# yakvrz/minesweeper-ppo

Hardware: NVIDIA B200
Metric: env_steps_per_s (higher is better)
Workload: dtype u32

## Files before the change

minesweeper_ppo_b200/csrc/msw_env.cu:

```cuda
#include "../../include/msw_b200.h"
#include "msw_common.cuh"
#include "msw_error.h"

#include <cuda_runtime.h>
#include <stdint.h>
#include <stdlib.h>
#include <string.h>


namespace msw {

void expand_obs_host(int H, int W, const uint32_t *mines, const uint32_t *revealed, const int32_t *meta, long long n,
                     float *obs, uint8_t *mask, uint64_t *shadow, int shadow_valid, int threads);

struct EnvParams {
    int H, W, HW, wpb;
    int mine_count, safe;
    float r_step, r_loss, r_win;
    uint32_t k0, k1;
    uint32_t thresh16;
    long long env_id_base;
    long long n;
    uint32_t *mines, *revealed, *flags;
    int4 *meta;
    const int32_t *a32;
    const long long *a64;
    const uint32_t *inj_bits;
    const uint8_t *inj_sel;
    float *reward;
    uint8_t *done;
    int8_t *outcome;
    int32_t *new_reveals, *step, *rcount;
    float *obs;
    uint8_t *mask;
    float *labels;
    uint8_t *valid;
    int rand_mode;
    uint32_t rk0, rk1, rand_step;
    int32_t *a_out;
    int vec_mode;
    long long seg_wa, seg_na, seg_wb, seg_nb;
    uint32_t g_valid[32], g_notcol0[32], g_notlast[32];
};

enum { MODE_STEP = 0, MODE_RESET = 1, MODE_ENCODE = 2 };

template <int CW, int CHW>
__device__ __noinline__ uint32_t sample_mines(const EnvParams &p, long long env_id, uint32_t episode,
                                              uint32_t startmask, int lane, const Geo &g)
{
    const int W = CW ? CW : p.W;
    const int HW = CHW ? CHW : p.HW;
    const int wpb = (HW + 31) >> 5;
    const int M = p.mine_count;
    uint32_t forb = startmask;
    if (p.safe) forb |= dilate8<CW>(startmask, lane, W, g);
    int allowed = HW - warp_popc_sum(forb);
    if (allowed < M) {
        forb = startmask;
        allowed = HW - 1;
    }
    const bool comp = 2 * M > allowed;
    const int K = comp ? allowed - M : M;
    const uint32_t thresh = CHW ? (65536u % (uint32_t)(CHW ? CHW : 1)) : p.thresh16;
    const uint32_t id_lo = (uint32_t)(unsigned long long)env_id;
    const uint32_t id_hi = (uint32_t)((unsigned long long)env_id >> 32);
    const uint32_t lt_mask = (1u << lane) - 1u;

    uint32_t chosen = 0;
    int cnt = 0;
    for (uint32_t batch = 0; cnt < K; ++batch) {
        uint32_t w[4];
        philox4x32_10(p.k0, p.k1, id_lo, id_hi, episode, batch * 32u + (uint32_t)lane, w);
#pragma unroll
        for (int r = 0; r < 8; ++r) {
            if (cnt >= K) break;
            const uint32_t x = (w[r >> 1] >> (16 * (r & 1))) & 0xFFFFu;
            const uint32_t m = x * (uint32_t)HW;
            const uint32_t d = m >> 16;
            const int owner = (int)(d >> 5);
            const uint32_t bit = 1u << (d & 31u);
            const uint32_t occ = __shfl_sync(FULL, forb | chosen, owner);
            const bool cand = ((m & 0xFFFFu) >= thresh) && !(occ & bit);
            const uint32_t same = __match_any_sync(FULL, cand ? d : (0x10000u + (uint32_t)lane));
            const bool novel = cand && ((same & lt_mask) == 0u);
            const uint32_t B = __ballot_sync(FULL, novel);
            const int need = K - cnt;
            const bool keep = novel && (__popc(B & lt_mask) < need);
            const int got = __popc(B);
            cnt += got < need ? got : need;
            for (int wd = 0; wd < wpb; ++wd) {
                const uint32_t nb = __reduce_or_sync(FULL, (keep && owner == wd) ? bit : 0u);
                if (lane == wd) chosen |= nb;
            }
        }
    }
    return comp ? (g.valid & ~forb & ~chosen) : chosen;
}

template <int CW, int CHW>
__device__ __forceinline__ void encode_board(const EnvParams &p, long long b, int lane, uint32_t R,
                                             uint32_t M, uint32_t F, int first, const Planes &pl,
                                             const Geo &g, const float4 *__restrict__ lut)
{
    const int HW = CHW ? CHW : p.HW;
    if (p.vec_mode == 1) {
        const int quads = HW >> 2;
        float4 *obs_b = p.obs ? reinterpret_cast<float4 *>(p.obs + b * (long long)(MSW_OBS_CHANNELS * HW)) : nullptr;
        uint32_t *mask_b = p.mask ? reinterpret_cast<uint32_t *>(p.mask + b * (long long)HW) : nullptr;
        float4 *lab_b = p.labels ? reinterpret_cast<float4 *>(p.labels + b * (long long)HW) : nullptr;
        uint32_t *val_b = p.valid ? reinterpret_cast<uint32_t *>(p.valid + b * (long long)HW) : nullptr;
        const uint32_t gate = first ? 15u : 0u;
#pragma unroll 2
        for (int q0 = 0; q0 < quads; q0 += 32) {
            const int q = q0 + lane;
            const bool act = q < quads;
            const int src = (act ? q : 0) >> 3;
            const int sh = (q & 7) << 2;
            const uint32_t r4 = (__shfl_sync(FULL, R, src) >> sh) & 15u;
            const uint32_t a0 = __shfl_sync(FULL, pl.c0, src) >> sh;
            const uint32_t a1 = __shfl_sync(FULL, pl.c1, src) >> sh;
            const uint32_t a2 = __shfl_sync(FULL, pl.c2, src) >> sh;
            const uint32_t a3 = __shfl_sync(FULL, pl.c3, src) >> sh;
            uint32_t l4 = 0, f4 = 0;
            if (lab_b) l4 = (__shfl_sync(FULL, M, src) >> sh) & gate;
            if (val_b && p.flags) f4 = (__shfl_sync(FULL, F, src) >> sh) & 15u;
            if (!act) continue;
            const uint32_t n4 = r4 ^ 15u;
            if (obs_b) {
                const uint32_t g4 = r4 & gate;
                float4 *o = obs_b + q;
                __stcs(o, lut[r4]);
#pragma unroll
                for (int k = 0; k < 9; ++k) {
                    const uint32_t lo = g4 & ((k & 1) ? a0 : ~a0) & ((k & 2) ? a1 : ~a1);
                    const uint32_t m = lo & ((k & 4) ? a2 : ~a2) & ((k & 8) ? a3 : ~a3);
                    __stcs(o + (1 + k) * quads, lut[m]);
                }
            }
            if (mask_b) __stcs(mask_b + q, nib_to_b4(n4));
            if (lab_b) __stcs(lab_b + q, lut[l4]);
            if (val_b) __stcs(val_b + q, nib_to_b4(n4 & ~f4 & gate));
        }
    } else {
        const uint32_t Lm = first ? M : 0u;
        const uint32_t Vm = first ? (~R & ~F & g.valid) : 0u;
        const int wpb = (HW + 31) >> 5;
        float *obs_b = p.obs ? p.obs + b * (long long)(MSW_OBS_CHANNELS * HW) : nullptr;
        uint8_t *mask_b = p.mask ? p.mask + b * (long long)HW : nullptr;
        float *lab_b = p.labels ? p.labels + b * (long long)HW : nullptr;
        uint8_t *val_b = p.valid ? p.valid + b * (long long)HW : nullptr;
        for (int it = 0; it < wpb; ++it) {
            const int cell = it * 32 + lane;
            const uint32_t r = (__shfl_sync(FULL, R, it) >> lane) & 1u;
            const uint32_t cnt = ((__shfl_sync(FULL, pl.c0, it) >> lane) & 1u) |
                                 (((__shfl_sync(FULL, pl.c1, it) >> lane) & 1u) << 1) |
                                 (((__shfl_sync(FULL, pl.c2, it) >> lane) & 1u) << 2) |
// ... 490 lines not shown
    g.notcol0 = p.g_notcol0[lane];
    g.notlast = p.g_notlast[lane];
    for (long long b = (long long)blockIdx.x * warps_per_block + (threadIdx.x >> 5); b < p.n; b += total_warps) {
        uint32_t M = 0, R = 0, F = 0;
        if (lane < wpb) {
            M = p.mines[b * wpb + lane];
            R = p.revealed[b * wpb + lane];
            if (p.flags) F = p.flags[b * wpb + lane];
        }
        const Planes pl = count_planes<0>(M, lane, p.W, g);
        for (int it = 0; it < wpb; ++it) {
            const int cell = it * 32 + lane;
            const uint32_t m = (__shfl_sync(FULL, M, it) >> lane) & 1u;
            const uint32_t r = (__shfl_sync(FULL, R, it) >> lane) & 1u;
            const uint32_t f = (__shfl_sync(FULL, F, it) >> lane) & 1u;
            const uint32_t cnt = ((__shfl_sync(FULL, pl.c0, it) >> lane) & 1u) |
                                 (((__shfl_sync(FULL, pl.c1, it) >> lane) & 1u) << 1) |
                                 (((__shfl_sync(FULL, pl.c2, it) >> lane) & 1u) << 2) |
                                 (((__shfl_sync(FULL, pl.c3, it) >> lane) & 1u) << 3);
            if (cell >= HW) continue;
            const long long o = b * (long long)HW + cell;
            if (q.o_mine) q.o_mine[o] = (uint8_t)m;
            if (q.o_rev) q.o_rev[o] = (uint8_t)r;
            if (q.o_flags) q.o_flags[o] = (uint8_t)f;
            if (q.o_counts) q.o_counts[o] = (uint8_t)cnt;
        }
    }
}

struct ActParams {
    const uint32_t *revealed;
    int HW, wpb;
    long long n, env_id_base;
    uint32_t k0, k1, step_index;
    int valid_only;
    int32_t *a32;
    long long *a64;
};

__global__ void __launch_bounds__(256) random_actions_kernel(const ActParams p)
{
    const long long b = (long long)blockIdx.x * blockDim.x + threadIdx.x;
    if (b >= p.n) return;
    const unsigned long long id = (unsigned long long)(p.env_id_base + b);
    uint32_t w[4];
    philox4x32_10(p.k0, p.k1 ^ 0x41435431u, (uint32_t)id, (uint32_t)(id >> 32), p.step_index, 0x5eedac71u, w);
    int action = 0;
    if (!p.valid_only) {
        action = (int)bounded(w, (uint32_t)p.HW);
    } else {
        const uint32_t *R = p.revealed + b * p.wpb;
        int cnt = 0;
        for (int i = 0; i < p.wpb; ++i) {
            uint32_t valid = (i == p.wpb - 1 && (p.HW & 31)) ? ((1u << (p.HW & 31)) - 1u) : 0xffffffffu;
            cnt += __popc(~R[i] & valid);
        }
        if (cnt > 0) {
            int k = (int)bounded(w, (uint32_t)cnt);
            for (int i = 0; i < p.wpb; ++i) {
                uint32_t valid = (i == p.wpb - 1 && (p.HW & 31)) ? ((1u << (p.HW & 31)) - 1u) : 0xffffffffu;
                const uint32_t free_cells = ~R[i] & valid;
                const int c = __popc(free_cells);
                if (k < c) {
                    action = i * 32 + (int)__fns(free_cells, 0, k + 1);
                    break;
                }
                k -= c;
            }
        }
    }
    if (p.a32) p.a32[b] = action;
    if (p.a64) p.a64[b] = action;
}

static int fill_geometry(EnvParams &p, const msw_env_desc *d, long long n)
{
    if (!d) return fail(MSW_ERR_NULL, "desc is NULL");
    if (d->H < 1 || d->W < 1 || d->W > 32 || (long long)d->H * d->W > MSW_MAX_CELLS)
        return fail(MSW_ERR_BAD_SHAPE, "board %dx%d unsupported (need 1<=W<=32, H*W<=%d)", d->H, d->W, MSW_MAX_CELLS);
    if (d->mine_count < 0 || d->mine_count > d->H * d->W - 1)
        return fail(MSW_ERR_BAD_SHAPE, "mine_count %d out of range for %dx%d", d->mine_count, d->H, d->W);
    if (n < 0) return fail(MSW_ERR_BAD_SHAPE, "n=%lld < 0", n);
    memset(&p, 0, sizeof(p));
    p.H = d->H; p.W = d->W; p.HW = d->H * d->W; p.wpb = (p.HW + 31) / 32;
    p.mine_count = d->mine_count; p.safe = d->safe_nbhd != 0;
    p.r_step = d->reward_step; p.r_loss = d->reward_loss; p.r_win = d->reward_win;
    p.k0 = (uint32_t)d->seed; p.k1 = (uint32_t)(d->seed >> 32);
    p.thresh16 = 65536u % (uint32_t)p.HW;
    p.env_id_base = d->env_id_base;
    p.n = n;
    for (int w = 0; w < 32; ++w) {
        uint32_t v = 0, a = 0, z = 0;
        for (int j = 0; j < 32; ++j) {
            const int cell = w * 32 + j;
            if (cell >= p.HW) break;
            const int col = cell % p.W;
            v |= 1u << j;
            if (col != 0) a |= 1u << j;
            if (col != p.W - 1) z |= 1u << j;
        }
        p.g_valid[w] = v; p.g_notcol0[w] = a; p.g_notlast[w] = z;
    }
    return MSW_OK;
}

static int fill_params(EnvParams &p, const msw_env_desc *d, const msw_state *st, long long n)
{
    if (!st) return fail(MSW_ERR_NULL, "state is NULL");
    if (!st->mines || !st->revealed || !st->meta) return fail(MSW_ERR_NULL, "state pointer is NULL");
    if (((uintptr_t)st->meta & 15u) != 0) return fail(MSW_ERR_ALIGN, "state.meta must be 16-byte aligned");
    const int rc = fill_geometry(p, d, n);
    if (rc) return rc;
    p.mines = st->mines; p.revealed = st->revealed; p.flags = st->flags;
    p.meta = reinterpret_cast<int4 *>(st->meta);
    return MSW_OK;
}

static int set_encode_out(EnvParams &p, const msw_encode_out *out, bool require)
{
    if (!out) return require ? fail(MSW_ERR_NULL, "encode outputs are NULL") : MSW_OK;
    p.obs = out->obs; p.mask = out->mask; p.labels = out->mine_labels; p.valid = out->mine_valid;
    const uintptr_t f = (uintptr_t)p.obs | (uintptr_t)p.labels, m = (uintptr_t)p.mask | (uintptr_t)p.valid;
    p.vec_mode = 0;
    if ((p.HW & 3) == 0) {
        if ((f & 15u) || (m & 3u))
            return fail(MSW_ERR_ALIGN, "obs/mine_labels must be 16-byte and mask/mine_valid 4-byte aligned");
        p.vec_mode = 1;
    }
    return MSW_OK;
}

struct LaunchShape { int block, bpw; };

static inline LaunchShape launch_shape_cfg()
{
#ifdef MSW_DEV_KNOBS
    static const LaunchShape c = [] {
        auto env_int = [](const char *name, int dflt) { const char *e = getenv(name); return e ? atoi(e) : dflt; };
        LaunchShape v;
        int blk = env_int("MSW_BLOCK", 32);
        if (blk < 32) blk = 32;
        if (blk > 256) blk = 256;
        v.block = blk & ~31;
        v.bpw = env_int("MSW_BPW", 3);
        if (v.bpw < 1) v.bpw = 1;
        return v;
    }();
    return c;
#else
    return LaunchShape{32, 3};
#endif
}

static inline int grid_for(EnvParams &q, int resident_warps_per_sm, int *block_out)
{
    const LaunchShape c = launch_shape_cfg();
    const int wpc = c.block / 32;
    *block_out = c.block;
    const long long n = q.n;
    long long taper_pct = 200;
#ifdef MSW_DEV_KNOBS
    if (const char *e = getenv("MSW_TAPER_PCT")) taper_pct = atoll(e);
#endif
    const long long S = (long long)sm_count() * resident_warps_per_sm;
    long long n2 = 0, n1 = 0;
    if (c.bpw >= 3 && n >= 8 * S && taper_pct > 0) {
        n1 = S / 3 * taper_pct / 100;
        n2 = 2 * n1;
    }
    q.seg_na = n - n2 - n1;
    q.seg_wa = (q.seg_na + c.bpw - 1) / c.bpw;
    q.seg_nb = q.seg_na + n2;
    q.seg_wb = (n2 + 1) / 2;
    const long long warps = q.seg_wa + q.seg_wb + n1;
    long long blocks = (warps + wpc - 1) / wpc;
    if (blocks < 1) blocks = 1;
    if (blocks > 0x7fffffffLL) blocks = 0x7fffffffLL;
    return (int)blocks;
}

template <int MODE, int CW, int CHW>
static void launch_shape(const EnvParams &p, int grid, int block, cudaStream_t s)
{
    if (MODE != MODE_STEP)
        env_kernel<MODE, CW, CHW, false, 4><<<grid, block, 0, s>>>(p);
    else
        env_kernel<MODE, CW, CHW, true, 3><<<grid, block, 0, s>>>(p);
}

template <int MODE>
static int launch_env(const EnvParams &p_in, cudaStream_t s)
{
    if (p_in.n == 0) return MSW_OK;
    EnvParams p = p_in;
    int block = 256;
    const int grid = grid_for(p, MODE == MODE_STEP ? 24 : 32, &block);
    if (p.W == 16 && p.HW == 256)
        launch_shape<MODE, 16, 256>(p, grid, block, s);
    else if (p.W == 30 && p.HW == 480)
        launch_shape<MODE, 30, 480>(p, grid, block, s);
    else if (p.W == 16 && p.HW == 480)
        launch_shape<MODE, 16, 480>(p, grid, block, s);
    else
        launch_shape<MODE, 0, 0>(p, grid, block, s);
    MSW_CUDA_TRY(cudaGetLastError());
    return MSW_OK;
}

}

using namespace msw;

extern "C" int msw_reset(const msw_env_desc *desc, const msw_state *st, int64_t n,
                         const msw_encode_out *out, void *stream)
{
    EnvParams p;
    int rc = fill_params(p, desc, st, n);
    if (rc) return rc;
    if ((rc = set_encode_out(p, out, false))) return rc;
    return launch_env<MODE_RESET>(p, (cudaStream_t)stream);
}

extern "C" int msw_encode(const msw_env_desc *desc, const msw_state *st, int64_t n,
                          const msw_encode_out *out, void *stream)
{
    EnvParams p;
    int rc = fill_params(p, desc, st, n);
    if (rc) return rc;
    if ((rc = set_encode_out(p, out, true))) return rc;
    return launch_env<MODE_ENCODE>(p, (cudaStream_t)stream);
}

static int fill_step(EnvParams &p, const msw_env_desc *desc, const msw_state *st, const msw_step_io *io, int64_t n)
{
    int rc = fill_params(p, desc, st, n);
    if (rc) return rc;
    if (!io) return fail(MSW_ERR_NULL, "io is NULL");
    if (io->rand_mode < 0 || io->rand_mode > 2) return fail(MSW_ERR_ARG, "rand_mode must be 0, 1 or 2");
    if (!io->rand_mode && (io->actions32 != nullptr) == (io->actions64 != nullptr))
        return fail(MSW_ERR_ARG, "exactly one of actions32/actions64 must be set");
    if (!io->reward || !io->done) return fail(MSW_ERR_NULL, "reward/done outputs are required");
    if ((io->inject_sel != nullptr) != (io->inject_bits != nullptr))
        return fail(MSW_ERR_ARG, "inject_bits and inject_sel must be given together");
    p.a32 = io->actions32;
    p.a64 = reinterpret_cast<const long long *>(io->actions64);
    p.rand_mode = io->rand_mode; p.rand_step = io->rand_step;
    p.rk0 = (uint32_t)io->rand_seed; p.rk1 = (uint32_t)(io->rand_seed >> 32);
    p.a_out = io->actions_out32;
    p.inj_bits = io->inject_bits; p.inj_sel = io->inject_sel;
    p.reward = io->reward; p.done = io->done; p.outcome = io->outcome;
    p.new_reveals = io->new_reveals; p.step = io->step; p.rcount = io->revealed_count;
    return set_encode_out(p, &io->enc, false);
}

extern "C" int msw_step(const msw_env_desc *desc, const msw_state *st, const msw_step_io *io,
                        int64_t n, void *stream)
{
    EnvParams p;
    int rc = fill_step(p, desc, st, io, n);
    if (rc) return rc;
    return launch_env<MODE_STEP>(p, (cudaStream_t)stream);
}

extern "C" int msw_step_host(const msw_env_desc *desc, const msw_state *st, const msw_step_io *io,
                             const int32_t *h_actions32, const msw_host_out *h, int64_t n, void *stream)
{
    EnvParams p;
    int rc = fill_step(p, desc, st, io, n);
    if (rc) return rc;
    if (!h_actions32 || !io->actions32) return fail(MSW_ERR_NULL, "msw_step_host needs h_actions32 and io->actions32 staging");
    cudaStream_t s = (cudaStream_t)stream;
    const size_t N = (size_t)n, HW = (size_t)p.HW;

    struct Copy { void *dst; const void *src; size_t bytes; };
    Copy copies[8] = {};
    int nc = 0;
    auto d2h = [&](void *dst, const void *src, size_t bytes) {
        if (nc && (const char *)copies[nc - 1].src + copies[nc - 1].bytes == (const char *)src &&
            (char *)copies[nc - 1].dst + copies[nc - 1].bytes == (char *)dst)
            copies[nc - 1].bytes += bytes;
        else
            copies[nc++] = {dst, src, bytes};
    };
#define MSW_HOST_SCALAR(field, dev, type, bytes)                                                           \
    if (h && h->field) {                                                                                   \
        if (!(dev)) return fail(MSW_ERR_NULL, "host output " #field " requested without device staging"); \
        d2h(h->field, dev, bytes);                                                                         \
    }
    const bool expand = h && (h->obs || h->mask);
    const size_t wpb = (size_t)p.wpb;
    if (expand) {
        if (!h->stage) return fail(MSW_ERR_NULL, "msw_step_host: host obs/mask requested without the pinned state staging area");
        if (h->shadow && !(h->obs && h->mask))
            return fail(MSW_ERR_NULL, "msw_step_host: a shadow describes BOTH result arrays: obs and mask are required with it");
    }
    MSW_HOST_SCALAR(reward, p.reward, float, N * 4)
    MSW_HOST_SCALAR(done, p.done, uint8_t, N)
    MSW_HOST_SCALAR(outcome, p.outcome, int8_t, N)
    MSW_HOST_SCALAR(new_reveals, p.new_reveals, int32_t, N * 4)
    MSW_HOST_SCALAR(step, p.step, int32_t, N * 4)
    MSW_HOST_SCALAR(revealed_count, p.rcount, int32_t, N * 4)
#undef MSW_HOST_SCALAR

    MSW_CUDA_TRY(cudaMemcpyAsync(const_cast<int32_t *>(io->actions32), h_actions32, N * 4, cudaMemcpyHostToDevice, s));
    if ((rc = launch_env<MODE_STEP>(p, s))) return rc;
    for (int i = 0; i < nc; ++i)
        MSW_CUDA_TRY(cudaMemcpyAsync(copies[i].dst, copies[i].src, copies[i].bytes, cudaMemcpyDeviceToHost, s));
    if (!expand) {
        MSW_CUDA_TRY(cudaStreamSynchronize(s));
        return MSW_OK;
    }
    uint32_t *h_mines = reinterpret_cast<uint32_t *>(h->stage), *h_rev = h_mines + N * wpb;
    constexpr int MAX_SLICES = 4;
    const int slices = N >= 32768 ? MAX_SLICES : 1;
    const size_t per = ((N + slices - 1) / slices + 127) / 128 * 128;
    cudaEvent_t ev[MAX_SLICES] = {};
    int made = 0;
    cudaError_t err = cudaSuccess;
    for (int k = 0; k < slices && err == cudaSuccess; ++k) {
        const size_t lo = (size_t)k * per, hi = lo + per < N ? lo + per : N;
        if (lo >= hi) break;
        err = cudaMemcpyAsync(h_mines + lo * wpb, st->mines + lo * wpb, (hi - lo) * wpb * 4, cudaMemcpyDeviceToHost, s);
        if (err == cudaSuccess)
            err = cudaMemcpyAsync(h_rev + lo * wpb, st->revealed + lo * wpb, (hi - lo) * wpb * 4, cudaMemcpyDeviceToHost, s);
        if (err == cudaSuccess) err = cudaEventCreateWithFlags(&ev[k], cudaEventDisableTiming);
        if (err == cudaSuccess) {
            ++made;
            err = cudaEventRecord(ev[k], s);
        }
    }
    for (int k = 0; k < made && err == cudaSuccess; ++k) {
        const size_t lo = (size_t)k * per, hi = lo + per < N ? lo + per : N;
        err = cudaEventSynchronize(ev[k]);
        if (err == cudaSuccess)
            expand_obs_host(p.H, p.W, h_mines + lo * wpb, h_rev + lo * wpb, nullptr, (long long)(hi - lo),
                            h->obs ? h->obs + lo * MSW_OBS_CHANNELS * HW : nullptr, h->mask ? h->mask + lo * HW : nullptr,
                            h->shadow ? h->shadow + lo * (size_t)msw_shadow_words(p.H, p.W) : nullptr, h->shadow_valid, h->threads);
    }
    for (int k = 0; k < made; ++k) cudaEventDestroy(ev[k]);
    if (err != cudaSuccess) {
        cudaStreamSynchronize(s);
        return cuda_fail(err, "msw_step_host: state copy / expansion");
    }
    MSW_CUDA_TRY(cudaStreamSynchronize(s));
    return MSW_OK;
}

extern "C" int msw_unpack_state(const msw_env_desc *desc, const msw_state *st, int64_t n, uint8_t *mine,
                                uint8_t *revealed, uint8_t *flags, uint8_t *counts, void *stream)
{
    UnpackParams q;
    int rc = fill_params(q.e, desc, st, n);
    if (rc) return rc;
    q.o_mine = mine; q.o_rev = revealed; q.o_flags = flags; q.o_counts = counts;
    if (n == 0) return MSW_OK;
    unpack_kernel<<<(unsigned)((n + 7) / 8), 256, 0, (cudaStream_t)stream>>>(q);
    MSW_CUDA_TRY(cudaGetLastError());
    return MSW_OK;
}

extern "C" int msw_random_actions(const msw_env_desc *desc, const msw_state *st, int64_t n, uint64_t seed,
                                  uint32_t step_index, int32_t valid_only, int32_t *a32, int64_t *a64,
                                  void *stream)
{
    EnvParams e;
    int rc = fill_params(e, desc, st, n);
    if (rc) return rc;
    if (!a32 && !a64) return fail(MSW_ERR_NULL, "no action output given");
    if (n == 0) return MSW_OK;
    ActParams p;
    p.revealed = st->revealed; p.HW = e.HW; p.wpb = e.wpb; p.n = n; p.env_id_base = desc->env_id_base;
    p.k0 = (uint32_t)seed; p.k1 = (uint32_t)(seed >> 32); p.step_index = step_index;
    p.valid_only = valid_only; p.a32 = a32; p.a64 = reinterpret_cast<long long *>(a64);
    random_actions_kernel<<<(unsigned)((n + 255) / 256), 256, 0, (cudaStream_t)stream>>>(p);
    MSW_CUDA_TRY(cudaGetLastError());
    return MSW_OK;
}

extern "C" int msw_late_start(const msw_env_desc *desc, const msw_state *st, int64_t n, const uint8_t *sel,
                              uint64_t late_seed, float prob, int32_t min_hidden, int32_t max_hidden,
                              int32_t max_attempts, int32_t max_extra_steps, void *stream)
{
    LateParams q;
    int rc = fill_params(q.e, desc, st, n);
    if (rc) return rc;
    if (!(prob >= 0.0f) || min_hidden < 1 || max_hidden < min_hidden || max_attempts < 1 || max_extra_steps < 1)
        return fail(MSW_ERR_ARG, "msw_late_start: bad parameters (prob=%f hidden=[%d,%d] attempts=%d extra=%d)",
                    prob, min_hidden, max_hidden, max_attempts, max_extra_steps);
    if (n == 0 || prob <= 0.0f) return MSW_OK;
    q.sel = sel;
    q.lk0 = (uint32_t)late_seed; q.lk1 = (uint32_t)(late_seed >> 32);
    const double p24 = (double)prob * 16777216.0;
    q.prob24 = p24 >= 16777216.0 ? 16777216u : (uint32_t)p24;
    q.min_hidden = min_hidden; q.max_hidden = max_hidden;
    q.max_attempts = max_attempts; q.max_extra_steps = max_extra_steps;
    late_start_kernel<<<(unsigned)((n + 3) / 4), 128, 0, (cudaStream_t)stream>>>(q);
    MSW_CUDA_TRY(cudaGetLastError());
    return MSW_OK;
}

extern "C" int msw_gather_encode(const msw_env_desc *desc, const uint32_t *snap_mines, const uint32_t *snap_revealed,
                                 const uint32_t *snap_flags, const uint8_t *snap_first, int64_t rows_in,
                                 const int64_t *idx, int64_t m, const msw_encode_out *out, void *stream)
{
    if (!snap_mines || !snap_revealed || !snap_first || !idx) return fail(MSW_ERR_NULL, "msw_gather_encode: NULL pointer");
    if (rows_in < 1) return fail(MSW_ERR_BAD_SHAPE, "msw_gather_encode: rows_in=%lld", (long long)rows_in);
    GatherParams q;
    int rc = fill_geometry(q.e, desc, m);
    if (rc) return rc;
    if ((rc = set_encode_out(q.e, out, true))) return rc;
    q.e.flags = const_cast<uint32_t *>(snap_flags);
    q.s_mines = snap_mines; q.s_revealed = snap_revealed; q.s_flags = snap_flags; q.s_first = snap_first;
    q.idx = reinterpret_cast<const long long *>(idx); q.rows_in = rows_in;
    if (m == 0) return MSW_OK;
    long long blocks = (m + 7) / 8;
    const long long cap = (long long)sm_count() * 16;
    if (blocks > cap) blocks = cap;
    cudaStream_t st = (cudaStream_t)stream;
    if (q.e.W == 16 && q.e.HW == 256)
        gather_encode_kernel<16, 256><<<(unsigned)blocks, 256, 0, st>>>(q);
    else
        gather_encode_kernel<0, 0><<<(unsigned)blocks, 256, 0, st>>>(q);
    MSW_CUDA_TRY(cudaGetLastError());
    return MSW_OK;
}

extern "C" int msw_forced_subset(const msw_env_desc *desc, const msw_state *st, int64_t n, uint32_t *out_bits,
                                 void *stream)
{
    SubsetParams q;
    int rc = fill_params(q.e, desc, st, n);
    if (rc) return rc;
    if (!out_bits) return fail(MSW_ERR_NULL, "msw_forced_subset: out_bits is NULL");
    q.out = out_bits;
    if (n == 0) return MSW_OK;
    const size_t smem = 4 * (3 * (size_t)MSW_MAX_CELLS + 128);
    subset_reveal_kernel<<<(unsigned)((n + 3) / 4), 128, smem, (cudaStream_t)stream>>>(q);
    MSW_CUDA_TRY(cudaGetLastError());
    return MSW_OK;
}
```

minesweeper_ppo_b200/env.py:

```python
from __future__ import annotations

import ctypes as C
import os
from collections.abc import Sequence
from dataclasses import dataclass
from typing import Any, Dict, Optional, Tuple, Union

import numpy as np
import torch

from . import _lib

OBS_CHANNELS = _lib.OBS_CHANNELS
_OUTCOME_NAMES = (None, "win", "loss")
_raw_stream = getattr(torch._C, "_cuda_getCurrentRawStream", None)
try:
    _libc = C.CDLL(None, use_errno=True)
    _libc.madvise
except Exception:
    _libc = None


@dataclass
class EnvConfig:
# ... 453 lines not shown
        if _rand is None:
            if not isinstance(actions, torch.Tensor):
                actions = torch.as_tensor(np.asarray(actions))
            assert tuple(actions.shape) == (n,)
            if actions.dtype not in (torch.int32, torch.int64):
                actions = actions.to(torch.int64)
            actions = actions.to(dev).contiguous()
        o = out if out is not None else self._alloc_encode()
        rewards = o.rewards if o.rewards is not None else torch.empty((n,), dtype=torch.float32, device=dev)
        dones = o.dones if o.dones is not None else torch.empty((n,), dtype=torch.bool, device=dev)
        io = self._io
        if _rand is None:
            io.actions32 = actions.data_ptr() if actions.dtype == torch.int32 else None
            io.actions64 = actions.data_ptr() if actions.dtype == torch.int64 else None
            io.rand_mode, io.actions_out32 = 0, None
        else:
            mode, step_index, seed, a_out = _rand
            io.actions32 = io.actions64 = None
            io.rand_mode, io.rand_step, io.rand_seed = mode, step_index & 0xFFFFFFFF, seed & 0xFFFFFFFFFFFFFFFF
            io.actions_out32 = self._check(a_out, (n,), torch.int32, "actions_out")
        io.inject_bits, io.inject_sel = ((self._inject[0].data_ptr(), self._inject[1].data_ptr())
                                         if self._inject is not None else (None, None))
        io.reward = self._check(rewards, (n,), torch.float32, "rewards")
        io.done = self._check(dones, (n,), torch.bool, "dones")
        infos: Dict[str, Any] = {}
        if want_infos:
            it = self._info_tensors()
            io.outcome, io.new_reveals = it["outcome"].data_ptr(), it["new_reveals"].data_ptr()
            io.step, io.revealed_count = it["step"].data_ptr(), it["revealed_count"].data_ptr()
            infos = {"outcome_code": it["outcome"], "last_new_reveals": it["new_reveals"], "step": it["step"],
                     "revealed_count": it["revealed_count"], "done": dones}
        else:
            io.outcome = io.new_reveals = io.step = io.revealed_count = None
        self._fill_encode(io.enc, o)
        with torch.cuda.device(dev):
            if self._late is None:
                _lib.check(self._L.msw_step(C.byref(self._desc), C.byref(self._state), C.byref(io), n,
                                            self._stream()), "msw_step")
            else:
                enc = _lib.EncodeOut(io.enc.obs, io.enc.mask, io.enc.mine_labels, io.enc.mine_valid)
                io.enc.obs = io.enc.mask = io.enc.mine_labels = io.enc.mine_valid = None
                _lib.check(self._L.msw_step(C.byref(self._desc), C.byref(self._state), C.byref(io), n,
                                            self._stream()), "msw_step")
                self._apply_late(io.done, enc)
        self._inject = None
        self._cache = None
        self.mine_labels, self.mine_valid = o.mine_labels, o.mine_valid
        return {"obs": o.obs, "action_mask": o.action_mask}, rewards, dones, infos

    def _host_buffers(self) -> Tuple[Dict[str, torch.Tensor], Dict[str, torch.Tensor]]:
        if not self._pinned:
            n, dev = self.num_envs, self.device
            spec = {
                "actions": ((n,), torch.int32), "reward": ((n,), torch.float32), "done": ((n,), torch.bool),
                "outcome": ((n,), torch.int8), "new_reveals": ((n,), torch.int32), "step": ((n,), torch.int32),
                "revealed_count": ((n,), torch.int32),
            }
            scalars = ("reward", "done", "outcome", "new_reveals", "step", "revealed_count")
            offs, off = {}, 0
            for k in scalars:
                shape, dt = spec[k]
                off = (off + dt.itemsize - 1) // dt.itemsize * dt.itemsize
                offs[k] = off
                off += n * dt.itemsize
            dev_blob = torch.empty((off,), dtype=torch.uint8, device=dev)
            pin_blob = _fastest_pinned(off, dev_blob, to_host=True)
            for k, (shape, dt) in spec.items():
                if k in offs:
                    nb = n * dt.itemsize
                    self._pinned[k] = pin_blob[offs[k]:offs[k] + nb].view(dt)
                    self._staging["h_" + k] = dev_blob[offs[k]:offs[k] + nb].view(dt)
                else:
                    self._staging["h_" + k] = torch.empty(shape, dtype=dt, device=dev)
                    self._pinned[k] = _fastest_pinned(n * dt.itemsize, self._staging["h_" + k].view(torch.uint8),
                                                      to_host=False).view(dt)
            self._pinned["stage"] = torch.empty((n * (2 * self.wpb + 4),), dtype=torch.int32).pin_memory()
        return self._pinned, self._staging

    @staticmethod
    def host_obs_d2h_bytes(H: int, W: int, n: int) -> int:
        wpb = (H * W + 31) // 32
        return n * (2 * wpb * 4 + 5)

    def _result_arrays(self) -> "_ResultSet":
        import sys
        for e in self._result_pool:
            if sys.getrefcount(e.obs) <= 2 and sys.getrefcount(e.raw) <= 3 and sys.getrefcount(e.mask) <= 2:
                return e
        e = _ResultSet(self.num_envs, self.H, self.W, self._L.msw_shadow_words(self.H, self.W))
        if len(self._result_pool) < 4:
            self._result_pool.append(e)
        return e

    def step_host(self, actions_pinned: torch.Tensor, *, copy_obs: bool = True, copy_infos: bool = True,
                  out: Optional[Tuple[np.ndarray, np.ndarray]] = None, threads: int = 0) -> Dict[str, Any]:
        n = self.num_envs
        pin, st = self._host_buffers()
        ap = actions_pinned.data_ptr()
        if ap not in self._pinned_ok:
            base = actions_pinned.untyped_storage().data_ptr()
            if not (actions_pinned.dtype == torch.int32 and tuple(actions_pinned.shape) == (n,) and
                    actions_pinned.is_contiguous() and (base in self._pinned_ok or actions_pinned.is_pinned())):
                raise ValueError("step_host: actions must be a pinned contiguous int32 [num_envs] CPU tensor")
            if len(self._pinned_ok) < 65536:
                self._pinned_ok.add(ap)
                self._pinned_ok.add(base)
        key = (copy_obs, copy_infos, self.aux_maps)
        prepared = self._host_calls.get(key)
        if prepared is None:
            io = _lib.StepIO()
            io.actions32, io.actions64 = st["h_actions"].data_ptr(), None
            io.rand_mode, io.actions_out32 = 0, None
            io.reward, io.done = st["h_reward"].data_ptr(), st["h_done"].data_ptr()
            io.outcome, io.new_reveals = st["h_outcome"].data_ptr(), st["h_new_reveals"].data_ptr()
            io.step, io.revealed_count = st["h_step"].data_ptr(), st["h_revealed_count"].data_ptr()
            if copy_obs:
                io.enc.obs = io.enc.mask = None
            else:
                if "h_obs" not in st:
                    st["h_obs"] = torch.empty((n, OBS_CHANNELS, self.H, self.W), dtype=torch.float32, device=self.device)
                    st["h_mask"] = torch.empty((n, self.HW), dtype=torch.bool, device=self.device)
                io.enc.obs, io.enc.mask = st["h_obs"].data_ptr(), st["h_mask"].data_ptr()
            if self.aux_maps:
                if "h_labels" not in st:
                    st["h_labels"] = torch.empty((n, self.H, self.W), dtype=torch.float32, device=self.device)
                    st["h_valid"] = torch.empty((n, self.H, self.W), dtype=torch.bool, device=self.device)
                io.enc.mine_labels, io.enc.mine_valid = st["h_labels"].data_ptr(), st["h_valid"].data_ptr()
            else:
                io.enc.mine_labels = io.enc.mine_valid = None
            h = _lib.HostOut()
            h.reward, h.done = pin["reward"].data_ptr(), pin["done"].data_ptr()
            if copy_infos:
                h.outcome, h.new_reveals = pin["outcome"].data_ptr(), pin["new_reveals"].data_ptr()
                h.step, h.revealed_count = pin["step"].data_ptr(), pin["revealed_count"].data_ptr()
            h.stage = pin["stage"].data_ptr()
            prepared = self._host_calls[key] = (io, h, C.byref(self._desc), C.byref(self._state), C.byref(io),
                                                C.byref(h))
        io, h, r_desc, r_state, r_io, r_h = prepared
        res: Dict[str, Any] = dict(pin)
        if not copy_obs:
            res["obs_device"], res["mask_device"] = st["h_obs"], st["h_mask"]
        rset = None
        if copy_obs:
            if out is not None:
                obs, mask = out
            else:
                rset = self._result_arrays()
                obs, mask = rset.obs, rset.mask
            if (obs.dtype != np.float32 or obs.shape != (n, OBS_CHANNELS, self.H, self.W) or not obs.flags.c_contiguous
                    or mask.dtype != np.bool_ or mask.shape != (n, self.HW) or not mask.flags.c_contiguous):
                raise ValueError("step_host: out must be (float32 [n,10,H,W], bool [n,HW]) C-contiguous arrays")
            h.obs, h.mask = obs.ctypes.data, mask.ctypes.data
            res["obs"], res["mask"] = obs, mask
        else:
            h.obs = h.mask = None
        use_shadow = rset is not None and self.host_delta
        if use_shadow:
            h.shadow, h.shadow_valid = rset.shadow.ctypes.data, rset.valid
        else:
            h.shadow, h.shadow_valid = None, 0
        if rset is not None:
            rset.valid = 0
        h.threads = int(threads) if threads else self.host_threads
        io.inject_bits, io.inject_sel = ((self._inject[0].data_ptr(), self._inject[1].data_ptr())
                                         if self._inject is not None else (None, None))
        if torch.cuda.current_device() == self.device.index:
            rc = self._L.msw_step_host(r_desc, r_state, r_io, ap, r_h, n, self._stream())
        else:
            with torch.cuda.device(self.device):
                rc = self._L.msw_step_host(r_desc, r_state, r_io, ap, r_h, n, self._stream())
        if rc:
            _lib.check(rc, "msw_step_host")
        if use_shadow:
            rset.valid = 1
        self._inject = None
        self._cache = None
        if self.aux_maps:
            self.mine_labels, self.mine_valid = st["h_labels"], st["h_valid"]
        return res

    def _step_numpy(self, actions) -> Tuple[Dict[str, np.ndarray], np.ndarray, np.ndarray, Dict[str, Any]]:
        n = self.num_envs
        actions = np.asarray(actions)
        assert actions.shape == (n,)
        if self._late is not None:
            a = np.mod(actions.astype(np.int64, copy=False), self.HW)
            self.api = "torch"
            try:
                b, r, d, info = self.step(torch.from_numpy(a))
            finally:
                self.api = "numpy"
            dones = d.cpu().numpy()
            outcome, newr = info["outcome_code"].cpu().numpy(), info["last_new_reveals"].cpu().numpy()
            step, rc = info["step"].cpu().numpy(), info["revealed_count"].cpu().numpy()
            batch = {"obs": b["obs"].cpu().numpy(), "action_mask": b["action_mask"].cpu().numpy()}
            rewards = r.cpu().numpy()
        else:
            pin, _ = self._host_buffers()
            if actions.dtype.kind in "iu" and (actions.dtype.itemsize < 4 or actions.dtype == np.int32):
                pin["actions"].numpy()[:] = actions
            else:
                a = actions.astype(np.int64, copy=False)
                if a.size and (a.max() > 2**31 - 1 or a.min() < -2**31):
                    a = np.mod(a, self.HW)
                pin["actions"].numpy()[:] = a
            res = self.step_host(pin["actions"])
            rewards = pin["reward"].numpy().copy()
            dones = pin["done"].numpy().copy()
            outcome, newr = pin["outcome"].numpy(), pin["new_reveals"].numpy()
            step, rc = pin["step"].numpy(), pin["revealed_count"].numpy()
            batch = {"obs": res["obs"], "action_mask": res["mask"]}
            del res
        hw = max(1, self.HW)
        step, newr, rc, outcome, done_i = step.copy(), newr.copy(), rc.copy(), outcome.copy(), dones.copy()
        infos = {
            "aux": _LazyList(n, lambda i: {"step": int(step[i]), "last_new_reveals": int(newr[i]),
                                           "revealed_frac": int(rc[i]) / hw}),
            "outcome": _LazyList(n, lambda i: _OUTCOME_NAMES[outcome[i]]),
            "done": _LazyList(n, lambda i: bool(done_i[i])),
        }
        return batch, rewards, dones, infos

    @property
    def state_tensors(self) -> Dict[str, Optional[torch.Tensor]]:
        return {"mines": self._mines, "revealed": self._revealed, "flags": self._flags, "meta": self._meta}
```

Baseline: 614.8 million.

## Pipeline step_host across slices with per-slice H2D, kernel, and D2H streams

Splits msw_step_host into up to four env slices. Each slice's action upload, step kernel and result downloads run on dedicated priority streams with event dependencies, so transfers overlap with compute on other slices. Streams and events are created once per device and reused, which removes the per-call event creation and destruction. The kernel grid taper now uses the total wave size so sliced launches keep the tail shaping. The Python side also skips redundant ctypes field writes when obs is not copied. The cost is more launches and cross-stream synchronisation, plus a global mutex per device.

```diff
diff --git a/minesweeper_ppo_b200/csrc/msw_env.cu b/minesweeper_ppo_b200/csrc/msw_env.cu
--- a/minesweeper_ppo_b200/csrc/msw_env.cu
+++ b/minesweeper_ppo_b200/csrc/msw_env.cu
@@ -3,6 +3,7 @@
 #include "msw_error.h"
 
 #include <cuda_runtime.h>
+#include <mutex>
 #include <stdint.h>
 #include <stdlib.h>
 #include <string.h>
@@ -799,7 +800,7 @@
 #endif
 }
 
-static inline int grid_for(EnvParams &q, int resident_warps_per_sm, int *block_out)
+static inline int grid_for(EnvParams &q, int resident_warps_per_sm, long long wave_boards, int *block_out)
 {
     const LaunchShape c = launch_shape_cfg();
     const int wpc = c.block / 32;
@@ -811,9 +812,10 @@
 #endif
     const long long S = (long long)sm_count() * resident_warps_per_sm;
     long long n2 = 0, n1 = 0;
-    if (c.bpw >= 3 && n >= 8 * S && taper_pct > 0) {
+    if (c.bpw >= 3 && wave_boards >= 8 * S && taper_pct > 0) {
         n1 = S / 3 * taper_pct / 100;
         n2 = 2 * n1;
+        if (n1 + n2 > n) n1 = n2 = 0;
     }
     q.seg_na = n - n2 - n1;
     q.seg_wa = (q.seg_na + c.bpw - 1) / c.bpw;
@@ -836,12 +838,13 @@
 }
 
 template <int MODE>
-static int launch_env(const EnvParams &p_in, cudaStream_t s)
+static int launch_env(const EnvParams &p_in, cudaStream_t s, long long wave_boards = -1)
 {
     if (p_in.n == 0) return MSW_OK;
     EnvParams p = p_in;
     int block = 256;
-    const int grid = grid_for(p, MODE == MODE_STEP ? 24 : 32, &block);
+    if (wave_boards < 0) wave_boards = p.n;
+    const int grid = grid_for(p, MODE == MODE_STEP ? 24 : 32, wave_boards, &block);
     if (p.W == 16 && p.HW == 256)
         launch_shape<MODE, 16, 256>(p, grid, block, s);
     else if (p.W == 30 && p.HW == 480)
@@ -853,6 +856,72 @@
     MSW_CUDA_TRY(cudaGetLastError());
     return MSW_OK;
 }
+
+template <class T>
+static inline T *at(T *ptr, long long k) { return ptr ? ptr + k : ptr; }
+
+static EnvParams env_slice(const EnvParams &p, long long lo, long long hi)
+{
+    EnvParams q = p;
+    const long long wpb = p.wpb, HW = p.HW;
+    q.n = hi - lo;
+    q.env_id_base = p.env_id_base + lo;
+    q.mines = at(p.mines, lo * wpb); q.revealed = at(p.revealed, lo * wpb); q.flags = at(p.flags, lo * wpb);
+    q.meta = at(p.meta, lo);
+    q.a32 = at(p.a32, lo); q.a64 = at(p.a64, lo);
+    q.inj_bits = at(p.inj_bits, lo * wpb); q.inj_sel = at(p.inj_sel, lo);
+    q.reward = at(p.reward, lo); q.done = at(p.done, lo); q.outcome = at(p.outcome, lo);
+    q.new_reveals = at(p.new_reveals, lo); q.step = at(p.step, lo); q.rcount = at(p.rcount, lo);
+    q.obs = at(p.obs, lo * MSW_OBS_CHANNELS * HW); q.mask = at(p.mask, lo * HW);
+    q.labels = at(p.labels, lo * HW); q.valid = at(p.valid, lo * HW);
+    q.a_out = at(p.a_out, lo);
+    return q;
+}
+
+constexpr int STEP_HOST_SLICES = 4;
+constexpr int STEP_HOST_MAX_DEVICES = 64;
+
+struct StepHostPipe {
+    std::mutex mu;
+    bool made = false;
+    bool prio = false;
+    cudaStream_t s[STEP_HOST_SLICES] = {};
+    cudaEvent_t start = nullptr, h2d[STEP_HOST_SLICES] = {}, kern[STEP_HOST_SLICES] = {}, fin[STEP_HOST_SLICES] = {};
+};
+
+static cudaError_t make_pipe(StepHostPipe &pp)
+{
+    int least = 0, greatest = 0;
+    cudaError_t e = cudaDeviceGetStreamPriorityRange(&least, &greatest);
+    pp.prio = e == cudaSuccess && least - greatest + 1 >= STEP_HOST_SLICES;
+#ifdef MSW_DEV_KNOBS
+    if (const char *v = getenv("MSW_STEP_HOST_PLAIN")) pp.prio = pp.prio && atoi(v) == 0;
+#endif
+    for (int k = 0; k < STEP_HOST_SLICES && e == cudaSuccess; ++k)
+        e = cudaStreamCreateWithPriority(&pp.s[k], cudaStreamNonBlocking, pp.prio ? greatest + k : least);
+    if (e == cudaSuccess) e = cudaEventCreateWithFlags(&pp.start, cudaEventDisableTiming);
+    for (int k = 0; k < STEP_HOST_SLICES && e == cudaSuccess; ++k) {
+        e = cudaEventCreateWithFlags(&pp.h2d[k], cudaEventDisableTiming);
+        if (e == cudaSuccess) e = cudaEventCreateWithFlags(&pp.kern[k], cudaEventDisableTiming);
+        if (e == cudaSuccess) e = cudaEventCreateWithFlags(&pp.fin[k], cudaEventDisableTiming);
+    }
+    if (e != cudaSuccess) {
+        for (int k = 0; k < STEP_HOST_SLICES; ++k) {
+            if (pp.s[k]) cudaStreamDestroy(pp.s[k]);
+            if (pp.h2d[k]) cudaEventDestroy(pp.h2d[k]);
+            if (pp.kern[k]) cudaEventDestroy(pp.kern[k]);
+            if (pp.fin[k]) cudaEventDestroy(pp.fin[k]);
+            pp.s[k] = nullptr; pp.h2d[k] = pp.kern[k] = pp.fin[k] = nullptr;
+        }
+        if (pp.start) cudaEventDestroy(pp.start);
+        pp.start = nullptr;
+        return e;
+    }
+    pp.made = true;
+    return cudaSuccess;
+}
+
+static StepHostPipe g_step_host_pipes[STEP_HOST_MAX_DEVICES];
 
 }
 
@@ -917,79 +986,132 @@
     if (rc) return rc;
     if (!h_actions32 || !io->actions32) return fail(MSW_ERR_NULL, "msw_step_host needs h_actions32 and io->actions32 staging");
     cudaStream_t s = (cudaStream_t)stream;
-    const size_t N = (size_t)n, HW = (size_t)p.HW;
-
-    struct Copy { void *dst; const void *src; size_t bytes; };
-    Copy copies[8] = {};
-    int nc = 0;
-    auto d2h = [&](void *dst, const void *src, size_t bytes) {
-        if (nc && (const char *)copies[nc - 1].src + copies[nc - 1].bytes == (const char *)src &&
-            (char *)copies[nc - 1].dst + copies[nc - 1].bytes == (char *)dst)
-            copies[nc - 1].bytes += bytes;
-        else
-            copies[nc++] = {dst, src, bytes};
-    };
-#define MSW_HOST_SCALAR(field, dev, type, bytes)                                                           \
+    const size_t N = (size_t)n, HW = (size_t)p.HW, wpb = (size_t)p.wpb;
+
+    struct Scalar { void *dst; const void *src; size_t esz; };
+    Scalar scal[6];
+    int ns = 0;
+#define MSW_HOST_SCALAR(field, dev, esz)                                                                   \
     if (h && h->field) {                                                                                   \
         if (!(dev)) return fail(MSW_ERR_NULL, "host output " #field " requested without device staging"); \
-        d2h(h->field, dev, bytes);                                                                         \
-    }
+        scal[ns++] = {h->field, dev, esz};                                                                 \
+    }
+    MSW_HOST_SCALAR(reward, p.reward, 4)
+    MSW_HOST_SCALAR(done, p.done, 1)
+    MSW_HOST_SCALAR(outcome, p.outcome, 1)
+    MSW_HOST_SCALAR(new_reveals, p.new_reveals, 4)
+    MSW_HOST_SCALAR(step, p.step, 4)
+    MSW_HOST_SCALAR(revealed_count, p.rcount, 4)
+#undef MSW_HOST_SCALAR
     const bool expand = h && (h->obs || h->mask);
-    const size_t wpb = (size_t)p.wpb;
     if (expand) {
         if (!h->stage) return fail(MSW_ERR_NULL, "msw_step_host: host obs/mask requested without the pinned state staging area");
         if (h->shadow && !(h->obs && h->mask))
             return fail(MSW_ERR_NULL, "msw_step_host: a shadow describes BOTH result arrays: obs and mask are required with it");
     }
-    MSW_HOST_SCALAR(reward, p.reward, float, N * 4)
-    MSW_HOST_SCALAR(done, p.done, uint8_t, N)
-    MSW_HOST_SCALAR(outcome, p.outcome, int8_t, N)
-    MSW_HOST_SCALAR(new_reveals, p.new_reveals, int32_t, N * 4)
-    MSW_HOST_SCALAR(step, p.step, int32_t, N * 4)
-    MSW_HOST_SCALAR(revealed_count, p.rcount, int32_t, N * 4)
-#undef MSW_HOST_SCALAR
-
-    MSW_CUDA_TRY(cudaMemcpyAsync(const_cast<int32_t *>(io->actions32), h_actions32, N * 4, cudaMemcpyHostToDevice, s));
-    if ((rc = launch_env<MODE_STEP>(p, s))) return rc;
-    for (int i = 0; i < nc; ++i)
-        MSW_CUDA_TRY(cudaMemcpyAsync(copies[i].dst, copies[i].src, copies[i].bytes, cudaMemcpyDeviceToHost, s));
-    if (!expand) {
-        MSW_CUDA_TRY(cudaStreamSynchronize(s));
-        return MSW_OK;
-    }
-    uint32_t *h_mines = reinterpret_cast<uint32_t *>(h->stage), *h_rev = h_mines + N * wpb;
-    constexpr int MAX_SLICES = 4;
-    const int slices = N >= 32768 ? MAX_SLICES : 1;
-    const size_t per = ((N + slices - 1) / slices + 127) / 128 * 128;
-    cudaEvent_t ev[MAX_SLICES] = {};
-    int made = 0;
+
+    int dev = 0;
+    MSW_CUDA_TRY(cudaGetDevice(&dev));
+    if (dev < 0 || dev >= STEP_HOST_MAX_DEVICES)
+        return fail(MSW_ERR_ARG, "msw_step_host: device %d (this library serves devices 0..%d)", dev, STEP_HOST_MAX_DEVICES - 1);
+    StepHostPipe &pp = g_step_host_pipes[dev];
+    std::lock_guard<std::mutex> lock(pp.mu);
+    if (!pp.made) {
+        const cudaError_t e = make_pipe(pp);
+        if (e != cudaSuccess) return cuda_fail(e, "msw_step_host: stream / event creation");
+    }
+
+    const int max_sl = N >= 32768 ? STEP_HOST_SLICES : 1;
+    const size_t per = ((N + max_sl - 1) / max_sl + 127) / 128 * 128;
+    const int nsl = per ? (int)((N + per - 1) / per) : 0;
+    cudaStream_t sh[STEP_HOST_SLICES], sk[STEP_HOST_SLICES], sd[STEP_HOST_SLICES];
+    for (int k = 0; k < nsl; ++k) {
+        if (nsl == 1) sh[k] = sk[k] = sd[k] = s;
+        else if (pp.prio) sh[k] = sk[k] = sd[k] = pp.s[k];
+        else sh[k] = pp.s[0], sk[k] = pp.s[1], sd[k] = pp.s[2];
+    }
+    sh[0] = s;
     cudaError_t err = cudaSuccess;
-    for (int k = 0; k < slices && err == cudaSuccess; ++k) {
+    const char *what = "";
+    auto ok = [&](cudaError_t e, const char *w) {
+        if (err == cudaSuccess && e != cudaSuccess) err = e, what = w;
+        return err == cudaSuccess;
+    };
+    auto drain = [&]() {
+        for (int k = 0; k < STEP_HOST_SLICES; ++k) cudaStreamSynchronize(pp.s[k]);
+        cudaStreamSynchronize(s);
+    };
+    bool entered[STEP_HOST_SLICES] = {};
+    auto enter = [&](cudaStream_t x) {
+        for (int j = 0; j < STEP_HOST_SLICES; ++j)
+            if (x == pp.s[j] && !entered[j]) {
+                entered[j] = true;
+                ok(cudaStreamWaitEvent(x, pp.start, 0), "wait start");
+            }
+    };
+    for (int k = 0; k < nsl && err == cudaSuccess; ++k) {
         const size_t lo = (size_t)k * per, hi = lo + per < N ? lo + per : N;
-        if (lo >= hi) break;
-        err = cudaMemcpyAsync(h_mines + lo * wpb, st->mines + lo * wpb, (hi - lo) * wpb * 4, cudaMemcpyDeviceToHost, s);
-        if (err == cudaSuccess)
-            err = cudaMemcpyAsync(h_rev + lo * wpb, st->revealed + lo * wpb, (hi - lo) * wpb * 4, cudaMemcpyDeviceToHost, s);
-        if (err == cudaSuccess) err = cudaEventCreateWithFlags(&ev[k], cudaEventDisableTiming);
-        if (err == cudaSuccess) {
-            ++made;
-            err = cudaEventRecord(ev[k], s);
-        }
-    }
-    for (int k = 0; k < made && err == cudaSuccess; ++k) {
+        enter(sh[k]);
+        ok(cudaMemcpyAsync(const_cast<int32_t *>(io->actions32) + lo, h_actions32 + lo, (hi - lo) * 4,
+                           cudaMemcpyHostToDevice, sh[k]), "actions H2D");
+        if (k == 0 && nsl > 1)
+            ok(cudaEventRecord(pp.start, s), "record start");
+        else if (sh[k] != sk[k] && ok(cudaEventRecord(pp.h2d[k], sh[k]), "record H2D"))
+            ok(cudaStreamWaitEvent(sk[k], pp.h2d[k], 0), "wait H2D");
+        enter(sk[k]);
+        if (err != cudaSuccess) break;
+        const long long wave = k == nsl - 1 ? (long long)N : pp.prio ? 0 : (long long)(hi - lo);
+        if ((rc = launch_env<MODE_STEP>(env_slice(p, (long long)lo, (long long)hi), sk[k], wave))) {
+            drain();
+            return rc;
+        }
+    }
+    uint32_t *h_mines = expand ? reinterpret_cast<uint32_t *>(h->stage) : nullptr;
+    uint32_t *h_rev = expand ? h_mines + N * wpb : nullptr;
+    int run_end[6];
+    for (int i = 0; i < ns;) {
+        int j = i + 1;
+        while (j < ns && (char *)scal[j - 1].dst + N * scal[j - 1].esz == (char *)scal[j].dst &&
+               (const char *)scal[j - 1].src + N * scal[j - 1].esz == (const char *)scal[j].src)
+            ++j;
+        run_end[i] = j;
+        i = j;
+    }
+    for (int k = 0; k < nsl && err == cudaSuccess; ++k) {
         const size_t lo = (size_t)k * per, hi = lo + per < N ? lo + per : N;
-        err = cudaEventSynchronize(ev[k]);
-        if (err == cudaSuccess)
+        const bool last = k == nsl - 1;
+        enter(sd[k]);
+        if (nsl > 1 && ok(cudaEventRecord(pp.kern[k], sk[k]), "record kernel"))
+            for (int j = last ? 0 : k; j <= k; ++j)
+                if (sk[j] != sd[k]) ok(cudaStreamWaitEvent(sd[k], pp.kern[j], 0), "wait kernel");
+        for (int i = 0; i < ns && err == cudaSuccess; i = run_end[i]) {
+            const int e = run_end[i] - 1;
+            char *dst = (char *)scal[i].dst + lo * scal[i].esz;
+            const char *src = (const char *)scal[i].src + lo * scal[i].esz;
+            const size_t bytes = last ? (size_t)((char *)scal[e].dst + N * scal[e].esz - dst) : (hi - lo) * scal[i].esz;
+            ok(cudaMemcpyAsync(dst, src, bytes, cudaMemcpyDeviceToHost, sd[k]), "scalars D2H");
+        }
+        if (expand && ok(cudaMemcpyAsync(h_mines + lo * wpb, st->mines + lo * wpb, (hi - lo) * wpb * 4,
+                                         cudaMemcpyDeviceToHost, sd[k]), "mines D2H"))
+            ok(cudaMemcpyAsync(h_rev + lo * wpb, st->revealed + lo * wpb, (hi - lo) * wpb * 4, cudaMemcpyDeviceToHost,
+                               sd[k]), "revealed D2H");
+        if (expand || sd[k] != s) ok(cudaEventRecord(pp.fin[k], sd[k]), "record slice end");
+    }
+    for (int k = 0; expand && k < nsl && err == cudaSuccess; ++k) {
+        const size_t lo = (size_t)k * per, hi = lo + per < N ? lo + per : N;
+        if (ok(cudaEventSynchronize(pp.fin[k]), "slice sync"))
             expand_obs_host(p.H, p.W, h_mines + lo * wpb, h_rev + lo * wpb, nullptr, (long long)(hi - lo),
                             h->obs ? h->obs + lo * MSW_OBS_CHANNELS * HW : nullptr, h->mask ? h->mask + lo * HW : nullptr,
                             h->shadow ? h->shadow + lo * (size_t)msw_shadow_words(p.H, p.W) : nullptr, h->shadow_valid, h->threads);
     }
-    for (int k = 0; k < made; ++k) cudaEventDestroy(ev[k]);
+    if (nsl > 1)
+        for (int k = 0; k < nsl && err == cudaSuccess; ++k) ok(cudaEventSynchronize(pp.fin[k]), "slice end sync");
+    else
+        ok(cudaStreamSynchronize(s), "stream sync");
     if (err != cudaSuccess) {
-        cudaStreamSynchronize(s);
-        return cuda_fail(err, "msw_step_host: state copy / expansion");
-    }
-    MSW_CUDA_TRY(cudaStreamSynchronize(s));
+        drain();
+        return cuda_fail(err, what);
+    }
     return MSW_OK;
 }
 
diff --git a/minesweeper_ppo_b200/env.py b/minesweeper_ppo_b200/env.py
--- a/minesweeper_ppo_b200/env.py
+++ b/minesweeper_ppo_b200/env.py
@@ -629,18 +629,19 @@
                 raise ValueError("step_host: out must be (float32 [n,10,H,W], bool [n,HW]) C-contiguous arrays")
             h.obs, h.mask = obs.ctypes.data, mask.ctypes.data
             res["obs"], res["mask"] = obs, mask
-        else:
-            h.obs = h.mask = None
         use_shadow = rset is not None and self.host_delta
         if use_shadow:
             h.shadow, h.shadow_valid = rset.shadow.ctypes.data, rset.valid
-        else:
+        elif copy_obs:
             h.shadow, h.shadow_valid = None, 0
         if rset is not None:
             rset.valid = 0
-        h.threads = int(threads) if threads else self.host_threads
-        io.inject_bits, io.inject_sel = ((self._inject[0].data_ptr(), self._inject[1].data_ptr())
-                                         if self._inject is not None else (None, None))
+        if copy_obs:
+            h.threads = int(threads) if threads else self.host_threads
+        if self._inject is not None:
+            io.inject_bits, io.inject_sel = self._inject[0].data_ptr(), self._inject[1].data_ptr()
+        elif io.inject_sel is not None:
+            io.inject_bits = io.inject_sel = None
         if torch.cuda.current_device() == self.device.index:
             rc = self._L.msw_step_host(r_desc, r_state, r_io, ap, r_h, n, self._stream())
         else:
```

Result: no change. 615.0 million, median of 6 (+0.0%).
